# THUDM/CogView

Hardware: AMD Instinct MI355X
Metric: train tokens/sec/node (seq1089, 4B GPT) at 1/2/4/8 MI355X; % MFMA roofline (higher is better)
Workload: dtype fp16

## Files before the change

### cogview_amd/csrc/attention.hip

```cpp
#include "common.cuh"
#include "cogview_hip.h"

#include <type_traits>

namespace {

constexpr int HD = 64;
constexpr int NT = 256;
constexpr float MASKED = -10000.0f;
constexpr int TILE = 8192;
#ifndef COGV_ATTN_STAGES
#define COGV_ATTN_STAGES 2
#endif
constexpr int NSTG = COGV_ATTN_STAGES;
static_assert(NSTG == 2 || NSTG == 3, "ring of two or three stages");
constexpr int COLSUM_SMEM = (128 * 68 + 256) * 4;

constexpr int DMA_TILE = 2;
template <int SIZE_, int DMAS_, bool COLSUM_> struct RingStage {
  static constexpr int SIZE = SIZE_, DMAS = DMAS_, INDEX = NSTG * SIZE_;
  static constexpr int dynamic_lds(int index_slots) {
    return ((COLSUM_ && INDEX < COLSUM_SMEM) ? COLSUM_SMEM : INDEX) + ((index_slots * 4 + 15) / 16) * 16;
  }
};
struct FwdStage : RingStage<2 * TILE, 2 * DMA_TILE, false> { static constexpr int K = 0, V = TILE; };
// ... 1 lines not shown
template <bool KB> struct DqStage : RingStage<2 * TILE + (KB ? 4 * DQ_KW_PITCH : 0), 2 * DMA_TILE + (KB ? 1 : 0), true> {
  static constexpr int K = 0, V = TILE, KW = 2 * TILE, KW_PITCH = DQ_KW_PITCH;
};
constexpr int DKDV_KW_PITCH = 272;
template <bool KB> struct DkdvStage : RingStage<2 * TILE + 512 + (KB ? 4 * DKDV_KW_PITCH : 256), 2 * DMA_TILE + 3, true> {
  static constexpr int Q = 0, DO = TILE, LSE = 2 * TILE, D = LSE + 256;
  static constexpr int RK = D + 256, KW = D + 256, KW_PITCH = DKDV_KW_PITCH;
};

struct AttnArgs {
  const void* q; const void* k; const void* v; void* o;
  const void* dout; void* dq; void* dk; void* dv;
  float* lse; float* dvec;
  float* colsum_ws;
  uint32_t* keepbits;
  const void* mask; long long mask_bs;
  const int* kv_index; long long kv_index_bs;
  long long kv_index_gs; int sp_w, sp_npiv; float sp_bias;
  long long q_bs, k_bs, v_bs, o_bs, do_bs, dq_bs, dk_bs, dv_bs;
  int q_rs, k_rs, v_rs, o_rs, do_rs, dq_rs, dk_rs, dv_rs;
  int B, H, s_q, s_k, sep_k;
  float scale;
  uint32_t thr16; float keep_scale; uint32_t rng_key;
};

struct BlockId { int bx, head, z; bool ok; };
__device__ __forceinline__ BlockId xcd_block_id(int nx, int H, int Z, bool heavy_last) {
  const int L = blockIdx.x, x = L & 7, j = L >> 3;
  const int ul = j / nx, k = j - ul * nx;
  const int u = ul * 8 + x;
  BlockId id;
  id.ok = u < H * Z;
  id.z = u / H; id.head = u - id.z * H;
  id.bx = heavy_last ? nx - 1 - k : k;
  return id;
}

typedef __attribute__((address_space(3))) void lds_void_t;
typedef __attribute__((address_space(1))) const void gbl_void_t;

template <int N> __device__ __forceinline__ void wait_vmcnt() { asm volatile("s_waitcnt vmcnt(%0)" ::"n"(N) : "memory"); }

__device__ __forceinline__ int aswz(int row) { return (((row >> 1) & 1) << 2) | ((row >> 2) & 3); }

template <typename T>
__device__ __forceinline__ void dma_tile(const T* base, long long rs, int row0, int nrows, char* lds, int wave, int lane,
// ... 132 lines not shown
  const int fr = lane & 31, fg = lane >> 5;
  float* row = lds + (wave * 32 + fr) * PITCH;
#pragma unroll
  for (int d = 0; d < 2; ++d)
#pragma unroll
    for (int gq = 0; gq < 4; ++gq)
      *reinterpret_cast<f32x4*>(row + 32 * d + 8 * gq + 4 * fg) =
          f32x4{vals[d][4 * gq], vals[d][4 * gq + 1], vals[d][4 * gq + 2], vals[d][4 * gq + 3]};
  __syncthreads();
  const int col = threadIdx.x & 63, slice = threadIdx.x >> 6;
  float s0 = 0.f, s1 = 0.f;
#pragma unroll
  for (int r = 0; r < 32; r += 2) {
    s0 += lds[(slice * 32 + r) * PITCH + col];
    s1 += lds[(slice * 32 + r + 1) * PITCH + col];
  }
  float* red = lds + 128 * PITCH;
  red[slice * 64 + col] = s0 + s1;
  __syncthreads();
  if (threadIdx.x < 64) dst[threadIdx.x] = red[threadIdx.x] + red[64 + threadIdx.x] + red[128 + threadIdx.x] + red[192 + threadIdx.x];
  __syncthreads();
}

template <bool IDX> __device__ __forceinline__ int* stage_index_table(const AttnArgs& p, int b, int gblk, char* behind_ring) {
  if (!(IDX && p.kv_index)) return nullptr;
  int* lidx = reinterpret_cast<int*>(behind_ring);
  const int* gi = p.kv_index + (long long)b * p.kv_index_bs + (long long)gblk * p.kv_index_gs;
  for (int i = threadIdx.x; i < p.s_k; i += NT) lidx[i] = gi[i];
  __syncthreads();
  return lidx;
}
struct SlotAttrs { unsigned long long masked, pivot; };
__device__ __forceinline__ SlotAttrs slot_attrs(const int* lidx, int kb, int lane, const AttnArgs& p) {
  int raw;
  const uint32_t ia = (uint32_t)(uintptr_t)(lidx + min(kb * 64 + lane, p.s_k - 1));
  asm volatile("ds_read_b32 %0, %1\n\ts_waitcnt lgkmcnt(0)" : "=v"(raw) : "v"(ia) : "memory");
  SlotAttrs a;
  a.masked = __ballot(raw < 0); a.pivot = __ballot(kb * 64 + lane < p.sp_npiv);
  return a;
}
__device__ __forceinline__ void apply_slot_attrs(f32x16& s, const SlotAttrs& a, int sb, int fg, float masked_raw, float bias_raw) {
  const uint32_t fm = (uint32_t)(a.masked >> (32 * sb)) >> (4 * fg), pm = (uint32_t)(a.pivot >> (32 * sb)) >> (4 * fg);
#pragma unroll
  for (int e = 0; e < 16; ++e) {
    const int bit = elem_idx(e);
    float v = s[e];
// ... 9 lines not shown
  for (int e = 0; e < 16; ++e) {
    const int key = kfirst + 4 * fg + elem_idx(e);
    mk[e] = HT<T>::to_f(mrow[min(key, p.s_k - 1)]);
    s[e] = fmaf(s[e], mk[e], masked_raw * (1.f - mk[e]));
  }
}
template <int NF> __device__ __forceinline__ void mask_edge(f32x16* s, int kfirst, int q0w, int myq, int off, int fg, const AttnArgs& p,
                                                            float masked_raw) {
  const bool all_visible = (kfirst + (32 * NF - 1) <= q0w + off) || (kfirst + (32 * NF - 1) < p.sep_k);
  if (!all_visible || kfirst + 32 * NF > p.s_k) {
#pragma unroll
    for (int sb = 0; sb < NF; ++sb) {
      const int base = kfirst + sb * 32 + 4 * fg;
      mask_frag(s[sb], myq + off - base, p.sep_k - base, p.s_k - base, masked_raw);
    }
  }
}

template <typename T, bool IDX, int DROP>
__global__ __launch_bounds__(NT, 2) void attn_fwd_kernel(const AttnArgs p) {
  const bool drop = DROP < 0 ? (p.thr16 != 0u) : (DROP != 0);
  extern __shared__ __attribute__((aligned(16))) char smem[];
  using L = FwdStage;
  const int lane = threadIdx.x & 63;
  const int wave = __builtin_amdgcn_readfirstlane(threadIdx.x >> 6);
  const int fr = lane & 31, fg = lane >> 5;
  const int nblk_x = (p.s_q + 127) >> 7;
  const BlockId bid = xcd_block_id(nblk_x, p.H, p.B, true);
  if (!bid.ok) return;
  const int b = bid.z, head = bid.head;
  const int q0 = bid.bx * 128, q0w = q0 + wave * 32;
  const bool spw = IDX && p.sp_w > 0;
  const int gblk = spw ? q0 / p.sp_w : 0;
  const int off = spw ? (p.s_k - p.sp_w - gblk * p.sp_w) : (p.s_k - p.s_q);
  const T* Q = reinterpret_cast<const T*>(p.q) + b * p.q_bs + head * HD;
  const T* K = reinterpret_cast<const T*>(p.k) + b * p.k_bs + head * HD;
  const T* V = reinterpret_cast<const T*>(p.v) + b * p.v_bs + head * HD;
  const int myq = q0w + fr;
  const bool wave_active = q0w < p.s_q;

  typename HT<T>::v8 qf[4];
#pragma unroll
  for (int t = 0; t < 4; ++t) qf[t] = load_frag_global<T>(Q + (long long)myq * p.q_rs + 16 * t + 8 * fg, myq < p.s_q);

  const int q_last = min(p.s_q, q0 + 128) - 1;
  const int kend_blk = min(p.s_k, max(q_last + off + 1, p.sep_k));
// ... 5 lines not shown
#pragma unroll
  for (int d = 0; d < 2; ++d)
#pragma unroll
    for (int e = 0; e < 16; ++e) oacc[d][e] = 0.f;
  float m_run = -INFINITY, l_run = 0.f;
  const float sl2 = p.scale * 1.4426950408889634f;
  const float masked_raw = MASKED / p.scale;
  const long long arow = ((long long)b * p.H + head) * p.s_q + myq;
  const RowKey cb = row_key(p.rng_key, (unsigned long long)arow);
  const float kofs = drop ? __builtin_amdgcn_logf(p.keep_scale) : 0.f;
  const uint32_t loff[2] = {tr_lane_off(0, lane) ^ tr_lane_fix(lane), tr_lane_off(1, lane) ^ tr_lane_fix(lane)};
  const uint32_t smem_addr = (uint32_t)(uintptr_t)smem;

  int* const lidx = stage_index_table<IDX>(p, b, gblk, smem + L::INDEX);
  const float sp_bias_raw = spw ? p.sp_bias / p.scale : 0.f;
  auto issue = [&](int kb, int st) {
    dma_tile<T>(K, p.k_rs, kb * 64, p.s_k, smem + st * L::SIZE + L::K, wave, lane, lidx);
    dma_tile<T>(V, p.v_rs, kb * 64, p.s_k, smem + st * L::SIZE + L::V, wave, lane, lidx);
  };
  static_assert(L::DMAS == 2 * DMA_TILE, "issue(): K tile, V tile");
  uint32_t* const kwp = DROP == 2 ? p.keepbits + ((((long long)b * p.H + head) * ((p.s_k + 63) >> 6)) * 2 + fg) * p.s_q + min(myq, p.s_q - 1) : nullptr;
  if (nkb > 0) { issue(0, 0); if (NSTG > 2) issue(nkb > 1 ? 1 : 0, 1); }
  int st = 0;
  for (int kb = 0; kb < nkb; ++kb) {
    wait_vmcnt<(NSTG - 2) * L::DMAS>();
    __builtin_amdgcn_s_barrier();
    issue(min(kb + NSTG - 1, nkb - 1), st == 0 ? NSTG - 1 : st - 1);
    if (kb * 64 < kend_w) {
      const char* lk = smem + st * L::SIZE + L::K;
      const uint32_t lv = smem_addr + st * L::SIZE + L::V;
      f32x16 sacc[2];
#pragma unroll
      for (int sb = 0; sb < 2; ++sb) {
#pragma unroll
        for (int e = 0; e < 16; ++e) sacc[sb][e] = 0.f;
#pragma unroll
        for (int t = 0; t < 4; ++t)
          sacc[sb] = HT<T>::mfma32(nat_frag<T>(lk, sb * 32 + fr, 2 * t + fg), qf[t], sacc[sb]);
      }
      TrRaw vr[2][2];
      tr_frags_issue<T, 0>(lv, loff, vr);
      if (IDX && lidx) {
        const SlotAttrs sa = slot_attrs(lidx, kb, lane, p);
#pragma unroll
        for (int sb = 0; sb < 2; ++sb) apply_slot_attrs(sacc[sb], sa, sb, fg, masked_raw, sp_bias_raw);
      }
      const int kfirst = kb * 64;
      if (IDX && p.mask) {
        float mk[16];
#pragma unroll
// ... 51 lines not shown
      TrRaw vr2[2][2];
      tr_wait(vr[0][0], vr[0][1]); tr_wait(vr[1][0], vr[1][1]);
      tr_frags_issue<T, 1>(lv, loff, vr2);
#pragma unroll
      for (int t = 0; t < 2; ++t) {
        float pe[8];
#pragma unroll
        for (int e = 0; e < 8; ++e) pe[e] = sacc[0][8 * t + e];
        const typename HT<T>::v8 pb = cvt8<T>(pe);
#pragma unroll
        for (int d = 0; d < 2; ++d) oacc[d] = HT<T>::mfma32(tr_pack<T>(vr[t][d]), pb, oacc[d]);
      }
      tr_wait(vr2[0][0], vr2[0][1]); tr_wait(vr2[1][0], vr2[1][1]);
#pragma unroll
      for (int t = 0; t < 2; ++t) {
        float pe[8];
#pragma unroll
        for (int e = 0; e < 8; ++e) pe[e] = sacc[1][8 * t + e];
        const typename HT<T>::v8 pb = cvt8<T>(pe);
#pragma unroll
        for (int d = 0; d < 2; ++d) oacc[d] = HT<T>::mfma32(tr_pack<T>(vr2[t][d]), pb, oacc[d]);
      }
    }
    st = (st == NSTG - 1) ? 0 : st + 1;
  }
  wait_vmcnt<0>();
  if (wave_active && myq < p.s_q) {
    const float l_tot = l_run + __shfl_xor(l_run, 32, 64);
    const float inv = (drop ? p.keep_scale : 1.0f) / l_tot;
    if (fg == 0 && p.lse) p.lse[((long long)b * p.H + head) * p.s_q + myq] = (m_run + __builtin_amdgcn_logf(l_tot) - kofs) * 0.6931471805599453f;
    T* O = reinterpret_cast<T*>(p.o) + b * p.o_bs + (long long)myq * p.o_rs + head * HD;
#pragma unroll
    for (int d = 0; d < 2; ++d)
#pragma unroll
      for (int gq = 0; gq < 4; ++gq) {
        u32x2 w;
        w[0] = pack2<T>(oacc[d][4 * gq] * inv, oacc[d][4 * gq + 1] * inv);
        w[1] = pack2<T>(oacc[d][4 * gq + 2] * inv, oacc[d][4 * gq + 3] * inv);
        *reinterpret_cast<u32x2*>(O + d * 32 + 8 * gq + 4 * fg) = w;
      }
  }
}

template <typename T, bool IDX, int DROP>
__global__ __launch_bounds__(NT, 2) void attn_bwd_dq_kernel(const AttnArgs p) {
  const bool drop = DROP < 0 ? (p.thr16 != 0u) : (DROP != 0);
  extern __shared__ __attribute__((aligned(16))) char smem[];
  constexpr bool KB = DROP == 2;
  using L = DqStage<KB>;
  const int lane = threadIdx.x & 63;
  const int wave = __builtin_amdgcn_readfirstlane(threadIdx.x >> 6);
  const int fr = lane & 31, fg = lane >> 5;
  const int nblk_x = (p.s_q + 127) >> 7;
  const BlockId bid = xcd_block_id(nblk_x, p.H, p.B, true);
  if (!bid.ok) return;
  const int b = bid.z, head = bid.head;
  const int q0 = bid.bx * 128, q0w = q0 + wave * 32;
  const bool spw = IDX && p.sp_w > 0;
  const int gblk = spw ? q0 / p.sp_w : 0;
  const int off = spw ? (p.s_k - p.sp_w - gblk * p.sp_w) : (p.s_k - p.s_q);
  const T* Q = reinterpret_cast<const T*>(p.q) + b * p.q_bs + head * HD;
  const T* K = reinterpret_cast<const T*>(p.k) + b * p.k_bs + head * HD;
  const T* V = reinterpret_cast<const T*>(p.v) + b * p.v_bs + head * HD;
  const T* DO = reinterpret_cast<const T*>(p.dout) + b * p.do_bs + head * HD;
  const int myq = q0w + fr;
  const bool qvalid = myq < p.s_q;
  const bool wave_active = q0w < p.s_q;

  typename HT<T>::v8 qf[4], dof[4];
#pragma unroll
  for (int t = 0; t < 4; ++t) {
    qf[t] = load_frag_global<T>(Q + (long long)myq * p.q_rs + 16 * t + 8 * fg, qvalid);
    dof[t] = load_frag_global<T>(DO + (long long)myq * p.do_rs + 16 * t + 8 * fg, qvalid);
  }
  const long long arow = ((long long)b * p.H + head) * p.s_q + myq;
  const RowKey cb = row_key(p.rng_key, (unsigned long long)arow);
  const float kscale = drop ? p.keep_scale : 1.0f;
  const float lse2 = qvalid ? p.lse[arow] * 1.4426950408889634f : 0.f;
  float dv = 0.f;
  {
    const T* Op = reinterpret_cast<const T*>(p.o) + b * p.o_bs + head * HD;
#pragma unroll
    for (int t = 0; t < 4; ++t) {
      const typename HT<T>::v8 of = load_frag_global<T>(Op + (long long)myq * p.o_rs + 16 * t + 8 * fg, qvalid);
#pragma unroll
      for (int e = 0; e < 8; ++e) dv = fmaf((float)dof[t][e], (float)of[e], dv);
    }
    dv += __shfl_xor(dv, 32, 64);
    if (qvalid && fg == 0) {
      p.dvec[arow] = -dv;
      if (!KB) reinterpret_cast<uint32_t*>(p.dvec)[(long long)p.B * p.H * p.s_q + arow] = cb.rk;
      else p.dvec[(long long)p.B * p.H * p.s_q + arow] = -lse2;
    }
  }
  const float sl2 = p.scale * 1.4426950408889634f;
  const float masked_raw = MASKED / p.scale;

  const int q_last = min(p.s_q, q0 + 128) - 1;
  const int kend_blk = min(p.s_k, max(q_last + off + 1, p.sep_k));
  const int nkb = (kend_blk + 63) >> 6;
  const int qw_last = min(p.s_q, q0w + 32) - 1;
  const int kend_w = wave_active ? min(p.s_k, max(qw_last + off + 1, p.sep_k)) : 0;

  f32x16 dqacc[2];
#pragma unroll
  for (int d = 0; d < 2; ++d)
#pragma unroll
    for (int e = 0; e < 16; ++e) dqacc[d][e] = 0.f;
  const uint32_t loff[2] = {tr_lane_off(0, lane) ^ tr_lane_fix(lane), tr_lane_off(1, lane) ^ tr_lane_fix(lane)};
  const uint32_t smem_addr = (uint32_t)(uintptr_t)smem;

  int* const lidx = stage_index_table<IDX>(p, b, gblk, smem + L::INDEX);
  const float sp_bias_raw = spw ? p.sp_bias / p.scale : 0.f;
  const uint32_t* KWQ = KB ? p.keepbits + ((long long)b * p.H + head) * ((p.s_k + 63) >> 6) * 2 * p.s_q + (long long)fg * p.s_q + min(myq, p.s_q - 1)
                           : nullptr;
  auto issue = [&](int kb, int st) {
    dma_tile<T>(K, p.k_rs, kb * 64, p.s_k, smem + st * L::SIZE + L::K, wave, lane, lidx);
    dma_tile<T>(V, p.v_rs, kb * 64, p.s_k, smem + st * L::SIZE + L::V, wave, lane, lidx);
    if (KB) __builtin_amdgcn_global_load_lds((gbl_void_t*)(KWQ + (long long)kb * 2 * p.s_q),
                                             (lds_void_t*)(smem + st * L::SIZE + L::KW + wave * L::KW_PITCH), 4, 0, 0);
  };
  static_assert(L::DMAS == 2 * DMA_TILE + (KB ? 1 : 0), "issue(): K tile, V tile, KB: the wave's keep words");
  if (nkb > 0) { issue(0, 0); if (NSTG > 2) issue(nkb > 1 ? 1 : 0, 1); }
  int st = 0;
  for (int kb = 0; kb < nkb; ++kb) {
    wait_vmcnt<(NSTG - 2) * L::DMAS>();
    __builtin_amdgcn_s_barrier();
    issue(min(kb + NSTG - 1, nkb - 1), st == 0 ? NSTG - 1 : st - 1);
    if (kb * 64 < kend_w) {
      const char* lk = smem + st * L::SIZE + L::K; const char* lv = smem + st * L::SIZE + L::V;
      const uint32_t lkt = smem_addr + st * L::SIZE + L::K;
      uint32_t kwv = 0u;
      if (KB) {
        const uint32_t ka = smem_addr + st * L::SIZE + L::KW + wave * L::KW_PITCH + lane * 4;
        asm volatile("ds_read_b32 %0, %1\n\ts_waitcnt lgkmcnt(0)" : "=v"(kwv) : "v"(ka) : "memory");
      }
      SlotAttrs sa = {0ull, 0ull};
      if (spw) sa = slot_attrs(lidx, kb, lane, p);
      auto half = [&](auto SBc) {
        constexpr int sb = decltype(SBc)::value;
        f32x16 sacc, pacc;
#pragma unroll
        for (int e = 0; e < 16; ++e) { sacc[e] = 0.f; pacc[e] = 0.f; }
#pragma unroll
        for (int t = 0; t < 4; ++t) {
          sacc = HT<T>::mfma32(nat_frag<T>(lk, sb * 32 + fr, 2 * t + fg), qf[t], sacc);
          pacc = HT<T>::mfma32(nat_frag<T>(lv, sb * 32 + fr, 2 * t + fg), dof[t], pacc);
        }
        TrRaw kr[2][2];
        tr_frags_issue<T, sb>(lkt, loff, kr);
        if (spw) apply_slot_attrs(sacc, sa, sb, fg, masked_raw, sp_bias_raw);
// ... 16 lines not shown
            const float pr = fast_exp2(fmaf(sacc[e], sl2, -lse2));
            float dp = pacc[e];
            if (KB) {
              uint32_t sx;
              asm("v_bfe_i32 %0, %1, %2, 1" : "=v"(sx) : "v"(kwv), "n"(31 - (sb * 16 + e)));
              dp = __uint_as_float(sx & __float_as_uint(dp));
            }
            else if (drop) dp = keep_of(r, i, p.thr16) ? dp : 0.f;
            ds[e] = pr * fmaf(dp, kscale, -dv);
            if (IDX && p.mask) ds[e] *= mk[e];
          }
        }
        tr_wait(kr[0][0], kr[0][1]); tr_wait(kr[1][0], kr[1][1]);
#pragma unroll
        for (int t = 0; t < 2; ++t) {
          const typename HT<T>::v8 dsb = cvt8<T>(ds + 8 * t);
#pragma unroll
          for (int d = 0; d < 2; ++d) dqacc[d] = HT<T>::mfma32(tr_pack<T>(kr[t][d]), dsb, dqacc[d]);
        }
      };
      half(std::integral_constant<int, 0>{});
      half(std::integral_constant<int, 1>{});
    }
    st = (st == NSTG - 1) ? 0 : st + 1;
  }
  wait_vmcnt<0>();
  float rq[2][16];
  {
    T* DQ = reinterpret_cast<T*>(p.dq) + b * p.dq_bs + (long long)myq * p.dq_rs + head * HD;
#pragma unroll
    for (int d = 0; d < 2; ++d)
#pragma unroll
      for (int gq = 0; gq < 4; ++gq) {
        u32x2 w;
        w[0] = pack2<T>(dqacc[d][4 * gq] * p.scale, dqacc[d][4 * gq + 1] * p.scale);
        w[1] = pack2<T>(dqacc[d][4 * gq + 2] * p.scale, dqacc[d][4 * gq + 3] * p.scale);
        if (qvalid) *reinterpret_cast<u32x2*>(DQ + d * 32 + 8 * gq + 4 * fg) = w;
#pragma unroll
        for (int i = 0; i < 4; ++i)
          rq[d][4 * gq + i] = qvalid ? bits_to_f<T>((uint16_t)(w[i >> 1] >> (16 * (i & 1)))) : 0.f;
      }
  }
  if (p.colsum_ws) {
    __syncthreads();
    float* dst = p.colsum_ws + ((size_t)b * nblk_x + bid.bx) * (size_t)(3 * p.H * HD) + head * HD;
    tile_colsum(rq, reinterpret_cast<float*>(smem), dst, lane, wave);
  }
}

#if defined(COGV_ATTN_TS)
__device__ unsigned long long g_attn_ts[1024 * 8];
#define ATS(k_) do { const unsigned long long t_ = __builtin_readcyclecounter(); ats[k_] += t_ - ats_last; ats_last = t_; } while (0)
#else
#define ATS(k_) do { } while (0)
#endif
template <typename T, bool IDX, int DROP>
__global__ __launch_bounds__(NT, 2) void attn_bwd_dkdv_kernel(const AttnArgs p) {
  const bool drop = DROP < 0 ? (p.thr16 != 0u) : (DROP != 0);
  extern __shared__ __attribute__((aligned(16))) char smem[];
  constexpr bool KB = DROP == 2;
  using L = DkdvStage<KB>;
#if defined(COGV_ATTN_TS)
  unsigned long long ats[8] = {0, 0, 0, 0, 0, 0, 0, 0};
  const unsigned long long ats_begin = __builtin_readcyclecounter();
  unsigned long long ats_last = ats_begin;
#endif
  const int lane = threadIdx.x & 63;
  const int wave = __builtin_amdgcn_readfirstlane(threadIdx.x >> 6);
  const int fr = lane & 31, fg = lane >> 5;
  const bool spw = IDX && p.sp_w > 0;
  const int nblk = spw ? p.s_q / p.sp_w : 1;
  const int nblk_x = (p.s_k + 127) >> 7;
  const BlockId bid = xcd_block_id(nblk_x, p.H, p.B * nblk, false);
  if (!bid.ok) return;
  const int zb = bid.z, head = bid.head;
  const int b = spw ? zb / nblk : zb, gblk = spw ? zb - b * nblk : 0;
  const int k0 = bid.bx * 128, k0w = k0 + wave * 32;
  const int off = spw ? (p.s_k - p.sp_w - gblk * p.sp_w) : (p.s_k - p.s_q);
  const int qlo = gblk * p.sp_w, qhi = spw ? qlo + p.sp_w : p.s_q;
  const T* Q = reinterpret_cast<const T*>(p.q) + b * p.q_bs + head * HD;
  const T* K = reinterpret_cast<const T*>(p.k) + b * p.k_bs + head * HD;
  const T* V = reinterpret_cast<const T*>(p.v) + b * p.v_bs + head * HD;
  const T* DO = reinterpret_cast<const T*>(p.dout) + b * p.do_bs + head * HD;
  const float* LSE = p.lse + ((long long)b * p.H + head) * p.s_q;
  const float* DV = p.dvec + ((long long)b * p.H + head) * p.s_q;
  const float* RK = DV + (long long)p.B * p.H * p.s_q;
  const int mykey = k0w + fr;
  const bool kvalid = mykey < p.s_k;
  const bool wave_active = k0w < p.s_k;

  int krow = mykey;
  bool kflag = false;
  if (IDX && p.kv_index) {
    const int raw = kvalid ? p.kv_index[(long long)b * p.kv_index_bs + (long long)gblk * p.kv_index_gs + mykey] : 0;
    kflag = raw < 0; krow = raw & 0x7fffffff;
  }
  typename HT<T>::v8 kf[4], vf[4];
#pragma unroll
  for (int t = 0; t < 4; ++t) {
    kf[t] = load_frag_global<T>(K + (long long)krow * p.k_rs + 16 * t + 8 * fg, kvalid);
    vf[t] = load_frag_global<T>(V + (long long)krow * p.v_rs + 16 * t + 8 * fg, kvalid);
  }
  const int qbeg_blk = (k0 < p.sep_k) ? qlo : max(qlo, k0 - off);
  const int qbeg_w = (k0w < p.sep_k) ? qlo : max(qlo, k0w - off);
  const int qb0 = qbeg_blk >> 6;
  const int nqb = (qhi + 63) >> 6;
  const float sp_add = (spw && mykey < p.sp_npiv) ? p.sp_bias / p.scale : 0.f;
  const float sl2 = p.scale * 1.4426950408889634f;
  const float l2e = 1.4426950408889634f;
  const float masked_raw = MASKED / p.scale;
  const long long arow0 = ((long long)b * p.H + head) * p.s_q;
  const float kscale = drop ? p.keep_scale : 1.0f;
  const uint32_t gweyl = (uint32_t)(mykey >> 2) * 0x9E3779B9u;

  f32x16 dkacc[2], dvacc[2];
#pragma unroll
  for (int d = 0; d < 2; ++d)
#pragma unroll
    for (int e = 0; e < 16; ++e) { dkacc[d][e] = 0.f; dvacc[d][e] = 0.f; }
  const uint32_t loff[2] = {tr_lane_off(0, lane) ^ tr_lane_fix(lane), tr_lane_off(1, lane) ^ tr_lane_fix(lane)};
  const uint32_t smem_addr = (uint32_t)(uintptr_t)smem;

  const int nkbt = (p.s_k + 63) >> 6;
  const uint32_t* KWS = KB ? p.keepbits + ((((long long)b * p.H + head) * nkbt + min((k0 >> 6) + (wave >> 1), nkbt - 1)) * 2 + (wave & 1)) * p.s_q
                           : nullptr;
  auto issue = [&](int qb, int st) {
    char* base = smem + st * L::SIZE;
    dma_tile<T>(Q, p.q_rs, qb * 64, p.s_q, base + L::Q, wave, lane);
    dma_tile<T>(DO, p.do_rs, qb * 64, p.s_q, base + L::DO, wave, lane);
    dma_stat(KB ? RK : LSE, qb * 64, p.s_q, base + L::LSE, lane);
    dma_stat(DV, qb * 64, p.s_q, base + L::D, lane);
    if (KB) dma_stat(reinterpret_cast<const float*>(KWS), qb * 64, p.s_q, base + L::KW + wave * L::KW_PITCH, lane);
    else dma_stat(RK, qb * 64, p.s_q, base + L::RK, lane);
  };
  static_assert(L::DMAS == 2 * DMA_TILE + 3, "issue(): Q tile, dO tile, LSE row, D row, row keys or the wave's keep-word segment");
  const int kr = mykey & 31;
  const uint32_t kw_seg = (uint32_t)(((wave >> 1) * 2 + ((kr >> 2) & 1)) * (L::KW_PITCH / 4));
  const uint32_t kw_bit = 31u - (uint32_t)((wave & 1) * 16 + 4 * (kr >> 3) + (kr & 3));
  if (qb0 < nqb) { issue(qb0, 0); if (NSTG > 2) issue(min(qb0 + 1, nqb - 1), 1); }
  int st = 0;
  ATS(4);
  for (int qb = qb0; qb < nqb; ++qb) {
    wait_vmcnt<(NSTG - 2) * L::DMAS>();
    __builtin_amdgcn_s_barrier();
    ATS(0);
    issue(min(qb + NSTG - 1, nqb - 1), st == 0 ? NSTG - 1 : st - 1);
    ATS(1);
#if defined(COGV_ATTN_TS)
    ats[6] += 1;
#endif
    if (wave_active && qb * 64 + 63 >= qbeg_w) {
      const char* lq = smem + st * L::SIZE + L::Q; const char* ldo = smem + st * L::SIZE + L::DO;
      const uint32_t lqt = smem_addr + st * L::SIZE + L::Q, ldot = smem_addr + st * L::SIZE + L::DO;
      const float* lse_row = reinterpret_cast<const float*>(smem + st * L::SIZE + L::LSE);
      const float* d_row = reinterpret_cast<const float*>(smem + st * L::SIZE + L::D);
      const uint32_t* rk_row = reinterpret_cast<const uint32_t*>(smem + st * L::SIZE + L::RK);
      const uint32_t* kw_segs = reinterpret_cast<const uint32_t*>(smem + st * L::SIZE + L::KW);
      auto half = [&](auto SBc) {
        constexpr int sb = decltype(SBc)::value;
        f32x16 sacc, pacc;
#pragma unroll
        for (int e = 0; e < 16; ++e) { sacc[e] = 0.f; pacc[e] = 0.f; }
        TrRaw dor_a[2][2], qr_a[2][2];
        if (KB) { tr_frags_issue<T, sb>(ldot, loff, dor_a); tr_frags_issue<T, sb>(lqt, loff, qr_a); }
#pragma unroll
        for (int t = 0; t < 4; ++t) {
          sacc = HT<T>::mfma32(nat_frag<T>(lq, sb * 32 + fr, 2 * t + fg), kf[t], sacc);
          pacc = HT<T>::mfma32(nat_frag<T>(ldo, sb * 32 + fr, 2 * t + fg), vf[t], pacc);
        }
        const int qfirst = qb * 64 + sb * 32;
        const bool all_visible = (qfirst >= k0w + 31 - off) || (k0w + 31 < p.sep_k);
        const bool tail = qfirst + 32 > p.s_q;
        if (!all_visible || tail) {
// ... 87 lines not shown
            for (int t = 0; t < 2; ++t)
#pragma unroll
              for (int d = 0; d < 2; ++d) dvacc[d] = HT<T>::mfma32(tr_pack<T>(dor[t][d]), pb[t], dvacc[d]);
          }
          {
            TrRaw qr[2][2];
            tr_frags_sync<T, sb>(lqt, loff, qr);
#pragma unroll
            for (int t = 0; t < 2; ++t)
#pragma unroll
              for (int d = 0; d < 2; ++d) dkacc[d] = HT<T>::mfma32(tr_pack<T>(qr[t][d]), dsb[t], dkacc[d]);
          }
        }
      };
      half(std::integral_constant<int, 0>{});
      half(std::integral_constant<int, 1>{});
    }
    ATS(2);
    st = (st == NSTG - 1) ? 0 : st + 1;
  }
  wait_vmcnt<0>();
  float rk[2][16], rv[2][16];
  {
    T* DK = reinterpret_cast<T*>(p.dk) + zb * p.dk_bs + (long long)mykey * p.dk_rs + head * HD;
    T* DVp = reinterpret_cast<T*>(p.dv) + zb * p.dv_bs + (long long)mykey * p.dv_rs + head * HD;
#pragma unroll
    for (int d = 0; d < 2; ++d)
#pragma unroll
      for (int gq = 0; gq < 4; ++gq) {
        u32x2 w, w2;
        w[0] = pack2<T>(dkacc[d][4 * gq] * p.scale, dkacc[d][4 * gq + 1] * p.scale);
        w[1] = pack2<T>(dkacc[d][4 * gq + 2] * p.scale, dkacc[d][4 * gq + 3] * p.scale);
        if (kvalid) *reinterpret_cast<u32x2*>(DK + d * 32 + 8 * gq + 4 * fg) = w;
        w2[0] = pack2<T>(dvacc[d][4 * gq], dvacc[d][4 * gq + 1]);
        w2[1] = pack2<T>(dvacc[d][4 * gq + 2], dvacc[d][4 * gq + 3]);
        if (kvalid) *reinterpret_cast<u32x2*>(DVp + d * 32 + 8 * gq + 4 * fg) = w2;
#pragma unroll
        for (int i = 0; i < 4; ++i) {
          rk[d][4 * gq + i] = kvalid ? bits_to_f<T>((uint16_t)(w[i >> 1] >> (16 * (i & 1)))) : 0.f;
          rv[d][4 * gq + i] = kvalid ? bits_to_f<T>((uint16_t)(w2[i >> 1] >> (16 * (i & 1)))) : 0.f;
        }
      }
  }
  if (p.colsum_ws) {
    __syncthreads();
    float* dst = p.colsum_ws + ((size_t)zb * nblk_x + bid.bx) * (size_t)(3 * p.H * HD) + (size_t)p.H * HD + head * HD;
    tile_colsum(rk, reinterpret_cast<float*>(smem), dst, lane, wave);
    tile_colsum(rv, reinterpret_cast<float*>(smem), dst + (size_t)p.H * HD, lane, wave);
  }
#if defined(COGV_ATTN_TS)
  ATS(3);
  if (lane == 0) {
    ats[5] = __builtin_readcyclecounter() - ats_begin; ats[7] = 1;
#pragma unroll
    for (int k = 0; k < 8; ++k) atomicAdd(&g_attn_ts[(((blockIdx.x << 2) + wave) & 1023) * 8 + k], ats[k]);
  }
#endif
}

struct DecodeArgs {
  const void* qkv; void* cache; void* out; const long long* pos; float* ws; int* tickets;
  long long qkv_bs, cache_bs, out_bs; int cache_rs;
  int B, H, cap, nsplit; float scale_l2e;
  const int* first;
};
template <typename T, bool RAGGED = false>
__global__ __launch_bounds__(256) void attn_decode_kernel(const DecodeArgs p) {
  __shared__ float red_o[32][64];
  __shared__ float red_m[4], red_l[32];
  const int t = threadIdx.x, dch = t & 7, kg = t >> 3, lane = t & 63, wave = t >> 6;
  const int split = blockIdx.x, head = blockIdx.y, b = blockIdx.z;
  const int hp = p.H * HD;
  const T* qrow = reinterpret_cast<const T*>(p.qkv) + b * p.qkv_bs + head * HD + dch * 8;
  float q8[8], kn[8], vn[8];
  unpack8<T>(*reinterpret_cast<const u32x4*>(qrow), q8);
  const u32x4 knew = *reinterpret_cast<const u32x4*>(qrow + hp), vnew = *reinterpret_cast<const u32x4*>(qrow + 2 * hp);
  T* crow = reinterpret_cast<T*>(p.cache) + b * p.cache_bs + head * HD + dch * 8;
  float sc[4]; u32x4 v8[4], kc8[4];
  float m_loc = -INFINITY;
  int first_b = 0;
// ... 202 lines not shown
      if (d->s_q != d->s_k || ((uintptr_t)d->colsum_partial & 15)) return COGV_ERR_ARG;
      a.colsum_ws = d->colsum_partial;
    }
    if (!aligned16(a.q) || !aligned16(a.k) || !aligned16(a.v) || !aligned16(a.o) || !aligned16(a.dout) ||
        !aligned16(a.dq) || !aligned16(a.dk) || !aligned16(a.dv)) return COGV_ERR_ARG;
    if ((a.q_rs | a.k_rs | a.v_rs | a.o_rs | a.do_rs | a.dq_rs | a.dk_rs | a.dv_rs) & 7) return COGV_ERR_ARG;
    if ((a.q_bs | a.k_bs | a.v_bs | a.o_bs | a.do_bs | a.dq_bs | a.dk_bs | a.dv_bs) & 7) return COGV_ERR_ARG;
  }
  const int slots = a.kv_index ? a.s_k : 0;
  pl.planes = a.sp_w > 0 && backward ? a.B * (a.s_q / a.sp_w) : a.B;
  pl.grid_q = 8u * (unsigned)((a.H * a.B + 7) / 8) * (unsigned)((a.s_q + 127) / 128);
  pl.grid_k = backward ? 8u * (unsigned)((a.H * pl.planes + 7) / 8) * (unsigned)((a.s_k + 127) / 128) : 0u;
  pl.lds_q = backward ? DqStage<false>::dynamic_lds(slots) : FwdStage::dynamic_lds(slots);
  pl.lds_k = backward ? DkdvStage<false>::dynamic_lds(0) : 0;
  if (pl.lds_q > 160 * 1024) return COGV_ERR_UNSUPPORTED;
  const bool drop = a.thr16 != 0u;
  pl.form = (a.kv_index || a.mask) ? ATTN_FLEXIBLE : drop ? ATTN_DENSE_DROP : ATTN_DENSE;
  if (d->keep_bits && drop && !a.kv_index) {
    if ((uintptr_t)d->keep_bits & 3) return COGV_ERR_ARG;
    a.keepbits = reinterpret_cast<uint32_t*>(d->keep_bits);
    pl.form = ATTN_DENSE_BITS;
    if (backward) { pl.lds_q = DqStage<true>::dynamic_lds(0); pl.lds_k = DkdvStage<true>::dynamic_lds(0); }
  }
  return COGV_OK;
}

template <void (*KERNEL)(const AttnArgs)>
void attn_launch(unsigned grid, int lds, hipStream_t st, const AttnArgs& a) {
  static int raised = 0;
  if (lds > raised) {
    (void)hipFuncSetAttribute(reinterpret_cast<const void*>(KERNEL), hipFuncAttributeMaxDynamicSharedMemorySize, lds);
    raised = lds;
  }
  hipLaunchKernelGGL(KERNEL, dim3(grid), dim3(NT), lds, st, a);
}
template <typename T, bool IDX, int DROP>
void attn_launch_form(const AttnPlan& pl, bool backward, hipStream_t st) {
  if (!backward) return attn_launch<attn_fwd_kernel<T, IDX, DROP>>(pl.grid_q, pl.lds_q, st, pl.a);
  attn_launch<attn_bwd_dq_kernel<T, IDX, DROP>>(pl.grid_q, pl.lds_q, st, pl.a);
  attn_launch<attn_bwd_dkdv_kernel<T, IDX, DROP>>(pl.grid_k, pl.lds_k, st, pl.a);
}
template <typename T>
void attn_launch_dtype(const AttnPlan& pl, bool backward, hipStream_t st) {
  switch (pl.form) {
    case ATTN_DENSE: return attn_launch_form<T, false, 0>(pl, backward, st);
    case ATTN_DENSE_DROP: return attn_launch_form<T, false, 1>(pl, backward, st);
// ... 80 lines not shown
                                       int B, int s, int H, int window, int times, int n_pivots, void* stream) {
  if (dtype != COGV_F16 && dtype != COGV_BF16) return COGV_ERR_UNSUPPORTED;
  if (!dk_slots || !dv_slots || !pivot_inv || !dk || !dv) return COGV_ERR_ARG;
  if (B <= 0 || s <= 0 || H <= 0 || window <= 0 || times <= 0 || n_pivots < 0 || (s % window)) return COGV_ERR_ARG;
  if (!aligned16(dk_slots) || !aligned16(dv_slots) || !aligned16(dk) || !aligned16(dv)) return COGV_ERR_ARG;
  if ((dk_bs | dv_bs | dk_rs | dv_rs) & 7) return COGV_ERR_ARG;
  const int C8 = H * HD / 8;
  const long long total = (long long)B * s * C8;
  const unsigned blocks = (unsigned)((total + 255) / 256);
  hipStream_t st = reinterpret_cast<hipStream_t>(stream);
  if (dtype == COGV_F16)
    hipLaunchKernelGGL((sparse_slot_reduce_kernel<f16_t>), dim3(blocks), dim3(256), 0, st, (const f16_t*)dk_slots,
                       (const f16_t*)dv_slots, pivot_inv, (f16_t*)dk, (f16_t*)dv, dk_bs, dk_rs, dv_bs, dv_rs, B, s, C8,
                       window, times, n_pivots);
  else
    hipLaunchKernelGGL((sparse_slot_reduce_kernel<bf16_t>), dim3(blocks), dim3(256), 0, st, (const bf16_t*)dk_slots,
                       (const bf16_t*)dv_slots, pivot_inv, (bf16_t*)dk, (bf16_t*)dv, dk_bs, dk_rs, dv_bs, dv_rs, B, s, C8,
                       window, times, n_pivots);
  return cogv_check_launch();
}

#if defined(COGV_ATTN_TS)
extern "C" int cogv_debug_attn_ts(unsigned long long* host_out, int reset) {
  static unsigned long long h[1024 * 8];
  if (host_out) {
    if (hipMemcpyFromSymbol(h, HIP_SYMBOL(g_attn_ts), sizeof(h)) != hipSuccess) return COGV_ERR_LAUNCH;
    for (int k = 0; k < 8; ++k) { host_out[k] = 0; for (int i = 0; i < 1024; ++i) host_out[k] += h[i * 8 + k]; }
  }
  if (reset) {
    for (int i = 0; i < 1024 * 8; ++i) h[i] = 0;
    if (hipMemcpyToSymbol(HIP_SYMBOL(g_attn_ts), h, sizeof(h)) != hipSuccess) return COGV_ERR_LAUNCH;
  }
  return COGV_OK;
}
#endif
```

Baseline: 42940.

## Stage attention backward row loads and dK/dV stores through LDS for coalesced access

In the dQ and dK/dV backward kernels, the per-row Q, dO, O, K and V fragments are now fetched with block-wide DMA tile copies into LDS and read back as fragments, instead of strided per-lane global loads. The dK/dV epilogue parks each wave's output in LDS and writes full coalesced 16-byte rows. The intent is to cut uncoalesced global traffic in prologues and epilogues. This costs extra barriers and LDS round trips. The path is on by default for non-flexible forms and can be turned off with an environment variable. The per-kernel timestamp instrumentation is also generalized across all three kernels, but it is compiled in only for debug builds.

```diff
diff --git a/cogview_amd/csrc/attention.hip b/cogview_amd/csrc/attention.hip
--- a/cogview_amd/csrc/attention.hip
+++ b/cogview_amd/csrc/attention.hip
@@ -1,6 +1,7 @@
 #include "common.cuh"
 #include "cogview_hip.h"
 
+#include <cstdlib>
 #include <type_traits>
 
 namespace {
@@ -48,6 +49,7 @@
   int B, H, s_q, s_k, sep_k;
   float scale;
   uint32_t thr16; float keep_scale; uint32_t rng_key;
+  int row_io;
 };
 
 struct BlockId { int bx, head, z; bool ok; };
@@ -226,6 +228,40 @@
   __syncthreads();
 }
 
+constexpr int ROWS_PITCH = 144;
+constexpr int ROWS_WAVE = 32 * ROWS_PITCH;
+template <typename T>
+__device__ __forceinline__ void store_rows_lds(char* park, T* tile, long long rs, int nvalid, const u32x2 (&w)[2][4], int lane) {
+  const int fr = lane & 31, fg = lane >> 5;
+#pragma unroll
+  for (int d = 0; d < 2; ++d)
+#pragma unroll
+    for (int gq = 0; gq < 4; ++gq) *reinterpret_cast<u32x2*>(park + fr * ROWS_PITCH + (4 * d + gq) * 16 + 8 * fg) = w[d][gq];
+  __builtin_amdgcn_wave_barrier();
+#pragma unroll
+  for (int j = 0; j < 4; ++j) {
+    const int row = 8 * j + (lane >> 3);
+    const u32x4 v = *reinterpret_cast<const u32x4*>(park + row * ROWS_PITCH + (lane & 7) * 16);
+    if (row < nvalid) *reinterpret_cast<u32x4*>(tile + row * rs + (lane & 7) * 8) = v;
+  }
+  __builtin_amdgcn_wave_barrier();
+}
+
+#if defined(COGV_ATTN_TS)
+__device__ unsigned long long g_attn_ts[3][1024 * 8];
+#define ATS_BEGIN unsigned long long ats[8] = {0, 0, 0, 0, 0, 0, 0, 0}; const unsigned long long ats_begin = __builtin_readcyclecounter(); \
+  unsigned long long ats_last = ats_begin
+#define ATS(k_) do { const unsigned long long t_ = __builtin_readcyclecounter(); ats[k_] += t_ - ats_last; ats_last = t_; } while (0)
+#define ATS_ITER ats[6] += 1
+#define ATS_END(kern_) do { ATS(3); if (lane == 0) { ats[5] = __builtin_readcyclecounter() - ats_begin; ats[7] = 1; \
+  for (int k_ = 0; k_ < 8; ++k_) atomicAdd(&g_attn_ts[kern_][(((blockIdx.x << 2) + wave) & 1023) * 8 + k_], ats[k_]); } } while (0)
+#else
+#define ATS_BEGIN do { } while (0)
+#define ATS(k_) do { } while (0)
+#define ATS_ITER do { } while (0)
+#define ATS_END(kern_) do { } while (0)
+#endif
+
 template <bool IDX> __device__ __forceinline__ int* stage_index_table(const AttnArgs& p, int b, int gblk, char* behind_ring) {
   if (!(IDX && p.kv_index)) return nullptr;
   int* lidx = reinterpret_cast<int*>(behind_ring);
@@ -281,6 +317,7 @@
   const bool drop = DROP < 0 ? (p.thr16 != 0u) : (DROP != 0);
   extern __shared__ __attribute__((aligned(16))) char smem[];
   using L = FwdStage;
+  ATS_BEGIN;
   const int lane = threadIdx.x & 63;
   const int wave = __builtin_amdgcn_readfirstlane(threadIdx.x >> 6);
   const int fr = lane & 31, fg = lane >> 5;
@@ -332,10 +369,14 @@
   uint32_t* const kwp = DROP == 2 ? p.keepbits + ((((long long)b * p.H + head) * ((p.s_k + 63) >> 6)) * 2 + fg) * p.s_q + min(myq, p.s_q - 1) : nullptr;
   if (nkb > 0) { issue(0, 0); if (NSTG > 2) issue(nkb > 1 ? 1 : 0, 1); }
   int st = 0;
+  ATS(4);
   for (int kb = 0; kb < nkb; ++kb) {
     wait_vmcnt<(NSTG - 2) * L::DMAS>();
     __builtin_amdgcn_s_barrier();
+    ATS(0);
     issue(min(kb + NSTG - 1, nkb - 1), st == 0 ? NSTG - 1 : st - 1);
+    ATS(1);
+    ATS_ITER;
     if (kb * 64 < kend_w) {
       const char* lk = smem + st * L::SIZE + L::K;
       const uint32_t lv = smem_addr + st * L::SIZE + L::V;
@@ -433,6 +474,7 @@
         for (int d = 0; d < 2; ++d) oacc[d] = HT<T>::mfma32(tr_pack<T>(vr2[t][d]), pb, oacc[d]);
       }
     }
+    ATS(2);
     st = (st == NSTG - 1) ? 0 : st + 1;
   }
   wait_vmcnt<0>();
@@ -451,6 +493,7 @@
         *reinterpret_cast<u32x2*>(O + d * 32 + 8 * gq + 4 * fg) = w;
       }
   }
+  ATS_END(0);
 }
 
 template <typename T, bool IDX, int DROP>
@@ -459,6 +502,7 @@
   extern __shared__ __attribute__((aligned(16))) char smem[];
   constexpr bool KB = DROP == 2;
   using L = DqStage<KB>;
+  ATS_BEGIN;
   const int lane = threadIdx.x & 63;
   const int wave = __builtin_amdgcn_readfirstlane(threadIdx.x >> 6);
   const int fr = lane & 31, fg = lane >> 5;
@@ -478,32 +522,6 @@
   const bool qvalid = myq < p.s_q;
   const bool wave_active = q0w < p.s_q;
 
-  typename HT<T>::v8 qf[4], dof[4];
-#pragma unroll
-  for (int t = 0; t < 4; ++t) {
-    qf[t] = load_frag_global<T>(Q + (long long)myq * p.q_rs + 16 * t + 8 * fg, qvalid);
-    dof[t] = load_frag_global<T>(DO + (long long)myq * p.do_rs + 16 * t + 8 * fg, qvalid);
-  }
-  const long long arow = ((long long)b * p.H + head) * p.s_q + myq;
-  const RowKey cb = row_key(p.rng_key, (unsigned long long)arow);
-  const float kscale = drop ? p.keep_scale : 1.0f;
-  const float lse2 = qvalid ? p.lse[arow] * 1.4426950408889634f : 0.f;
-  float dv = 0.f;
-  {
-    const T* Op = reinterpret_cast<const T*>(p.o) + b * p.o_bs + head * HD;
-#pragma unroll
-    for (int t = 0; t < 4; ++t) {
-      const typename HT<T>::v8 of = load_frag_global<T>(Op + (long long)myq * p.o_rs + 16 * t + 8 * fg, qvalid);
-#pragma unroll
-      for (int e = 0; e < 8; ++e) dv = fmaf((float)dof[t][e], (float)of[e], dv);
-    }
-    dv += __shfl_xor(dv, 32, 64);
-    if (qvalid && fg == 0) {
-      p.dvec[arow] = -dv;
-      if (!KB) reinterpret_cast<uint32_t*>(p.dvec)[(long long)p.B * p.H * p.s_q + arow] = cb.rk;
-      else p.dvec[(long long)p.B * p.H * p.s_q + arow] = -lse2;
-    }
-  }
   const float sl2 = p.scale * 1.4426950408889634f;
   const float masked_raw = MASKED / p.scale;
 
@@ -513,11 +531,6 @@
   const int qw_last = min(p.s_q, q0w + 32) - 1;
   const int kend_w = wave_active ? min(p.s_k, max(qw_last + off + 1, p.sep_k)) : 0;
 
-  f32x16 dqacc[2];
-#pragma unroll
-  for (int d = 0; d < 2; ++d)
-#pragma unroll
-    for (int e = 0; e < 16; ++e) dqacc[d][e] = 0.f;
   const uint32_t loff[2] = {tr_lane_off(0, lane) ^ tr_lane_fix(lane), tr_lane_off(1, lane) ^ tr_lane_fix(lane)};
   const uint32_t smem_addr = (uint32_t)(uintptr_t)smem;
 
@@ -532,12 +545,78 @@
                                              (lds_void_t*)(smem + st * L::SIZE + L::KW + wave * L::KW_PITCH), 4, 0, 0);
   };
   static_assert(L::DMAS == 2 * DMA_TILE + (KB ? 1 : 0), "issue(): K tile, V tile, KB: the wave's keep words");
-  if (nkb > 0) { issue(0, 0); if (NSTG > 2) issue(nkb > 1 ? 1 : 0, 1); }
+  const bool rows_in = !IDX && NSTG == 2 && p.row_io != 0;
+  const T* Op = reinterpret_cast<const T*>(p.o) + b * p.o_bs + head * HD;
+  const char* my_tile = smem + (wave >> 1) * TILE;
+  const int my_row = (wave & 1) * 32 + fr;
+  const typename HT<T>::v8 zero8 = load_frag_global<T>(Q, false);
+  typename HT<T>::v8 qf[4], dof[4], of[4];
+  if (rows_in) {
+    dma_tile<T>(Q, p.q_rs, q0, p.s_q, smem, wave, lane);
+    dma_tile<T>(Q, p.q_rs, q0 + 64, p.s_q, smem + TILE, wave, lane);
+    dma_tile<T>(DO, p.do_rs, q0, p.s_q, smem + L::SIZE, wave, lane);
+    dma_tile<T>(DO, p.do_rs, q0 + 64, p.s_q, smem + L::SIZE + TILE, wave, lane);
+    wait_vmcnt<0>();
+    __syncthreads();
+#pragma unroll
+    for (int t = 0; t < 4; ++t) {
+      qf[t] = nat_frag<T>(my_tile, my_row, 2 * t + fg);
+      dof[t] = nat_frag<T>(my_tile + L::SIZE, my_row, 2 * t + fg);
+    }
+    __syncthreads();
+    dma_tile<T>(Op, p.o_rs, q0, p.s_q, smem + L::SIZE, wave, lane);
+    dma_tile<T>(Op, p.o_rs, q0 + 64, p.s_q, smem + L::SIZE + TILE, wave, lane);
+    if (nkb > 0) { issue(0, 0); wait_vmcnt<L::DMAS>(); }
+    else wait_vmcnt<0>();
+    __builtin_amdgcn_s_barrier();
+#pragma unroll
+    for (int t = 0; t < 4; ++t) of[t] = nat_frag<T>(my_tile + L::SIZE, my_row, 2 * t + fg);
+    asm volatile("s_waitcnt lgkmcnt(0)" ::: "memory");
+#pragma unroll
+    for (int t = 0; t < 4; ++t) {
+      qf[t] = qvalid ? qf[t] : zero8; dof[t] = qvalid ? dof[t] : zero8; of[t] = qvalid ? of[t] : zero8;
+    }
+  } else {
+#pragma unroll
+    for (int t = 0; t < 4; ++t) {
+      qf[t] = load_frag_global<T>(Q + (long long)myq * p.q_rs + 16 * t + 8 * fg, qvalid);
+      dof[t] = load_frag_global<T>(DO + (long long)myq * p.do_rs + 16 * t + 8 * fg, qvalid);
+    }
+#pragma unroll
+    for (int t = 0; t < 4; ++t) of[t] = load_frag_global<T>(Op + (long long)myq * p.o_rs + 16 * t + 8 * fg, qvalid);
+  }
+  const long long arow = ((long long)b * p.H + head) * p.s_q + myq;
+  const RowKey cb = row_key(p.rng_key, (unsigned long long)arow);
+  const float kscale = drop ? p.keep_scale : 1.0f;
+  const float lse2 = qvalid ? p.lse[arow] * 1.4426950408889634f : 0.f;
+  float dv = 0.f;
+  {
+#pragma unroll
+    for (int t = 0; t < 4; ++t)
+#pragma unroll
+      for (int e = 0; e < 8; ++e) dv = fmaf((float)dof[t][e], (float)of[t][e], dv);
+    dv += __shfl_xor(dv, 32, 64);
+    if (qvalid && fg == 0) {
+      p.dvec[arow] = -dv;
+      if (!KB) reinterpret_cast<uint32_t*>(p.dvec)[(long long)p.B * p.H * p.s_q + arow] = cb.rk;
+      else p.dvec[(long long)p.B * p.H * p.s_q + arow] = -lse2;
+    }
+  }
+  f32x16 dqacc[2];
+#pragma unroll
+  for (int d = 0; d < 2; ++d)
+#pragma unroll
+    for (int e = 0; e < 16; ++e) dqacc[d][e] = 0.f;
+  if (!rows_in && nkb > 0) { issue(0, 0); if (NSTG > 2) issue(nkb > 1 ? 1 : 0, 1); }
   int st = 0;
+  ATS(4);
   for (int kb = 0; kb < nkb; ++kb) {
     wait_vmcnt<(NSTG - 2) * L::DMAS>();
     __builtin_amdgcn_s_barrier();
+    ATS(0);
     issue(min(kb + NSTG - 1, nkb - 1), st == 0 ? NSTG - 1 : st - 1);
+    ATS(1);
+    ATS_ITER;
     if (kb * 64 < kend_w) {
       const char* lk = smem + st * L::SIZE + L::K; const char* lv = smem + st * L::SIZE + L::V;
       const uint32_t lkt = smem_addr + st * L::SIZE + L::K;
@@ -600,6 +679,7 @@
       half(std::integral_constant<int, 0>{});
       half(std::integral_constant<int, 1>{});
     }
+    ATS(2);
     st = (st == NSTG - 1) ? 0 : st + 1;
   }
   wait_vmcnt<0>();
@@ -624,25 +704,16 @@
     float* dst = p.colsum_ws + ((size_t)b * nblk_x + bid.bx) * (size_t)(3 * p.H * HD) + head * HD;
     tile_colsum(rq, reinterpret_cast<float*>(smem), dst, lane, wave);
   }
-}
-
-#if defined(COGV_ATTN_TS)
-__device__ unsigned long long g_attn_ts[1024 * 8];
-#define ATS(k_) do { const unsigned long long t_ = __builtin_readcyclecounter(); ats[k_] += t_ - ats_last; ats_last = t_; } while (0)
-#else
-#define ATS(k_) do { } while (0)
-#endif
+  ATS_END(1);
+}
+
 template <typename T, bool IDX, int DROP>
 __global__ __launch_bounds__(NT, 2) void attn_bwd_dkdv_kernel(const AttnArgs p) {
   const bool drop = DROP < 0 ? (p.thr16 != 0u) : (DROP != 0);
   extern __shared__ __attribute__((aligned(16))) char smem[];
   constexpr bool KB = DROP == 2;
   using L = DkdvStage<KB>;
-#if defined(COGV_ATTN_TS)
-  unsigned long long ats[8] = {0, 0, 0, 0, 0, 0, 0, 0};
-  const unsigned long long ats_begin = __builtin_readcyclecounter();
-  unsigned long long ats_last = ats_begin;
-#endif
+  ATS_BEGIN;
   const int lane = threadIdx.x & 63;
   const int wave = __builtin_amdgcn_readfirstlane(threadIdx.x >> 6);
   const int fr = lane & 31, fg = lane >> 5;
@@ -674,10 +745,29 @@
     kflag = raw < 0; krow = raw & 0x7fffffff;
   }
   typename HT<T>::v8 kf[4], vf[4];
-#pragma unroll
-  for (int t = 0; t < 4; ++t) {
-    kf[t] = load_frag_global<T>(K + (long long)krow * p.k_rs + 16 * t + 8 * fg, kvalid);
-    vf[t] = load_frag_global<T>(V + (long long)krow * p.v_rs + 16 * t + 8 * fg, kvalid);
+  const bool rows_in = !IDX && NSTG == 2 && p.row_io != 0;
+  if (rows_in) {
+    dma_tile<T>(K, p.k_rs, k0, p.s_k, smem, wave, lane);
+    dma_tile<T>(K, p.k_rs, k0 + 64, p.s_k, smem + TILE, wave, lane);
+    dma_tile<T>(V, p.v_rs, k0, p.s_k, smem + L::SIZE, wave, lane);
+    dma_tile<T>(V, p.v_rs, k0 + 64, p.s_k, smem + L::SIZE + TILE, wave, lane);
+    wait_vmcnt<0>();
+    __syncthreads();
+    const typename HT<T>::v8 zero8 = load_frag_global<T>(K, false);
+#pragma unroll
+    for (int t = 0; t < 4; ++t) {
+      kf[t] = nat_frag<T>(smem + (wave >> 1) * TILE, (wave & 1) * 32 + fr, 2 * t + fg);
+      vf[t] = nat_frag<T>(smem + L::SIZE + (wave >> 1) * TILE, (wave & 1) * 32 + fr, 2 * t + fg);
+    }
+#pragma unroll
+    for (int t = 0; t < 4; ++t) { kf[t] = kvalid ? kf[t] : zero8; vf[t] = kvalid ? vf[t] : zero8; }
+    __syncthreads();
+  } else {
+#pragma unroll
+    for (int t = 0; t < 4; ++t) {
+      kf[t] = load_frag_global<T>(K + (long long)krow * p.k_rs + 16 * t + 8 * fg, kvalid);
+      vf[t] = load_frag_global<T>(V + (long long)krow * p.v_rs + 16 * t + 8 * fg, kvalid);
+    }
   }
   const int qbeg_blk = (k0 < p.sep_k) ? qlo : max(qlo, k0 - off);
   const int qbeg_w = (k0w < p.sep_k) ? qlo : max(qlo, k0w - off);
@@ -724,9 +814,7 @@
     ATS(0);
     issue(min(qb + NSTG - 1, nqb - 1), st == 0 ? NSTG - 1 : st - 1);
     ATS(1);
-#if defined(COGV_ATTN_TS)
-    ats[6] += 1;
-#endif
+    ATS_ITER;
     if (wave_active && qb * 64 + 63 >= qbeg_w) {
       const char* lq = smem + st * L::SIZE + L::Q; const char* ldo = smem + st * L::SIZE + L::DO;
       const uint32_t lqt = smem_addr + st * L::SIZE + L::Q, ldot = smem_addr + st * L::SIZE + L::DO;
@@ -860,25 +948,31 @@
   wait_vmcnt<0>();
   float rk[2][16], rv[2][16];
   {
-    T* DK = reinterpret_cast<T*>(p.dk) + zb * p.dk_bs + (long long)mykey * p.dk_rs + head * HD;
-    T* DVp = reinterpret_cast<T*>(p.dv) + zb * p.dv_bs + (long long)mykey * p.dv_rs + head * HD;
+    const int row_io = IDX ? 0 : p.row_io;
+    T* DK = reinterpret_cast<T*>(p.dk) + zb * p.dk_bs + head * HD;
+    T* DVp = reinterpret_cast<T*>(p.dv) + zb * p.dv_bs + head * HD;
+    u32x2 w[2][4], w2[2][4];
 #pragma unroll
     for (int d = 0; d < 2; ++d)
 #pragma unroll
       for (int gq = 0; gq < 4; ++gq) {
-        u32x2 w, w2;
-        w[0] = pack2<T>(dkacc[d][4 * gq] * p.scale, dkacc[d][4 * gq + 1] * p.scale);
-        w[1] = pack2<T>(dkacc[d][4 * gq + 2] * p.scale, dkacc[d][4 * gq + 3] * p.scale);
-        if (kvalid) *reinterpret_cast<u32x2*>(DK + d * 32 + 8 * gq + 4 * fg) = w;
-        w2[0] = pack2<T>(dvacc[d][4 * gq], dvacc[d][4 * gq + 1]);
-        w2[1] = pack2<T>(dvacc[d][4 * gq + 2], dvacc[d][4 * gq + 3]);
-        if (kvalid) *reinterpret_cast<u32x2*>(DVp + d * 32 + 8 * gq + 4 * fg) = w2;
+        w[d][gq][0] = pack2<T>(dkacc[d][4 * gq] * p.scale, dkacc[d][4 * gq + 1] * p.scale);
+        w[d][gq][1] = pack2<T>(dkacc[d][4 * gq + 2] * p.scale, dkacc[d][4 * gq + 3] * p.scale);
+        if (row_io == 0 && kvalid) *reinterpret_cast<u32x2*>(DK + (long long)mykey * p.dk_rs + d * 32 + 8 * gq + 4 * fg) = w[d][gq];
+        w2[d][gq][0] = pack2<T>(dvacc[d][4 * gq], dvacc[d][4 * gq + 1]);
+        w2[d][gq][1] = pack2<T>(dvacc[d][4 * gq + 2], dvacc[d][4 * gq + 3]);
+        if (row_io == 0 && kvalid) *reinterpret_cast<u32x2*>(DVp + (long long)mykey * p.dv_rs + d * 32 + 8 * gq + 4 * fg) = w2[d][gq];
 #pragma unroll
         for (int i = 0; i < 4; ++i) {
-          rk[d][4 * gq + i] = kvalid ? bits_to_f<T>((uint16_t)(w[i >> 1] >> (16 * (i & 1)))) : 0.f;
-          rv[d][4 * gq + i] = kvalid ? bits_to_f<T>((uint16_t)(w2[i >> 1] >> (16 * (i & 1)))) : 0.f;
+          rk[d][4 * gq + i] = kvalid ? bits_to_f<T>((uint16_t)(w[d][gq][i >> 1] >> (16 * (i & 1)))) : 0.f;
+          rv[d][4 * gq + i] = kvalid ? bits_to_f<T>((uint16_t)(w2[d][gq][i >> 1] >> (16 * (i & 1)))) : 0.f;
         }
       }
+    if (row_io != 0) {
+      __syncthreads();
+      store_rows_lds<T>(smem + wave * ROWS_WAVE, DK + (long long)k0w * p.dk_rs, p.dk_rs, p.s_k - k0w, w, lane);
+      store_rows_lds<T>(smem + wave * ROWS_WAVE, DVp + (long long)k0w * p.dv_rs, p.dv_rs, p.s_k - k0w, w2, lane);
+    }
   }
   if (p.colsum_ws) {
     __syncthreads();
@@ -886,14 +980,7 @@
     tile_colsum(rk, reinterpret_cast<float*>(smem), dst, lane, wave);
     tile_colsum(rv, reinterpret_cast<float*>(smem), dst + (size_t)p.H * HD, lane, wave);
   }
-#if defined(COGV_ATTN_TS)
-  ATS(3);
-  if (lane == 0) {
-    ats[5] = __builtin_readcyclecounter() - ats_begin; ats[7] = 1;
-#pragma unroll
-    for (int k = 0; k < 8; ++k) atomicAdd(&g_attn_ts[(((blockIdx.x << 2) + wave) & 1023) * 8 + k], ats[k]);
-  }
-#endif
+  ATS_END(2);
 }
 
 struct DecodeArgs {
@@ -1142,6 +1229,10 @@
     pl.form = ATTN_DENSE_BITS;
     if (backward) { pl.lds_q = DqStage<true>::dynamic_lds(0); pl.lds_k = DkdvStage<true>::dynamic_lds(0); }
   }
+  const char* row_io = getenv("COGV_ATTN_ROW_IO");
+  a.row_io = pl.form == ATTN_FLEXIBLE ? 0 : (row_io ? atoi(row_io) != 0 : 1);
+  static_assert(4 * ROWS_WAVE <= DkdvStage<false>::INDEX && 4 * ROWS_WAVE <= DkdvStage<true>::INDEX,
+                "store_rows_lds: the four waves' regions lie inside the dK.dV ring");
   return COGV_OK;
 }
 
@@ -1268,13 +1359,13 @@
 
 #if defined(COGV_ATTN_TS)
 extern "C" int cogv_debug_attn_ts(unsigned long long* host_out, int reset) {
-  static unsigned long long h[1024 * 8];
+  static unsigned long long h[3 * 1024 * 8];
   if (host_out) {
     if (hipMemcpyFromSymbol(h, HIP_SYMBOL(g_attn_ts), sizeof(h)) != hipSuccess) return COGV_ERR_LAUNCH;
-    for (int k = 0; k < 8; ++k) { host_out[k] = 0; for (int i = 0; i < 1024; ++i) host_out[k] += h[i * 8 + k]; }
+    for (int k = 0; k < 24; ++k) { host_out[k] = 0; for (int i = 0; i < 1024; ++i) host_out[k] += h[((k >> 3) * 1024 + i) * 8 + (k & 7)]; }
   }
   if (reset) {
-    for (int i = 0; i < 1024 * 8; ++i) h[i] = 0;
+    for (int i = 0; i < 3 * 1024 * 8; ++i) h[i] = 0;
     if (hipMemcpyToSymbol(HIP_SYMBOL(g_attn_ts), h, sizeof(h)) != hipSuccess) return COGV_ERR_LAUNCH;
   }
   return COGV_OK;
```

New measurement: 43240 (median of 6 runs). About the same (+0.7%).
